# iyioon/NYPC-Yacht-Auction

Measured on AMD Instinct MI355X. Metric: MCTS node-expansions/sec/GPU @4096 envs x100 sims; episodes/sec 1-8 GPU, higher is better.
Workload: dtype f32

## Files before the change

nypc-yacht-auction_amd/csrc/yk_engine.hip:

```cpp
#include <math.h>

#include <algorithm>
#include <vector>

#include "yk_api.h"
#include "yk_common.h"
#include "yk_net.h"

#define YK_MAX_GROUPS 8

using namespace yk;

namespace {

constexpr int MAXD = 64;
constexpr int LUT_N = 1 << 16;
constexpr int GAMES_PER_BLOCK = 4;
constexpr int GROUP_ALIGN = 16;
constexpr int YK_EXPAND_WPE = 4;
constexpr int RO_CAP = 3072;
constexpr int RO_K = 512;
constexpr int RV_CAP = 1024;
constexpr uint32_t RV_OFF = 0xFFFFFFFFu;

enum : uint32_t { T_INT = 0, T_F64 = 1, T_F32 = 2 };

struct NodeRec {
    uint64_t key[8];
    uint64_t hash;
    uint64_t vinfo;
    uint32_t p_off;
    uint32_t nvalid;
    uint32_t Ns;
    uint32_t pad;
};
struct Edge {
    double Q;
    uint32_t N;
    uint32_t tag;
};
__device__ __forceinline__ uint32_t edge_kind(uint32_t tag) { return tag & 3u; }
constexpr uint32_t PATH_DET = 0x80000000u;

constexpr int GST = 16;
struct EngDev {
    int E, NCAP, HCAP, ECAP, M, VCAP;
    int e_lo, e_hi;
    int T, dual;
    int64_t AE;
    int sims, temp_threshold;
    float c32;
    int prior;
    int fparts;
    int rec_pred, max_exp, rec_stride;
    int arena;
    int arena_agent, arena_opp;
    uint64_t seed;
    NodeRec* nodes[2];
    uint32_t* hidx[2];
    Edge* edges[2];
    uint32_t* node_count;
    uint32_t* edge_count;
    float* arenaP;
    uint16_t* arenaS;
    uint32_t* arena_top;
    uint8_t* gen;
    uint8_t* cur_round;
    uint4* root_c;
    int ro_k;
    uint32_t* rv;
    uint16_t* ro_j;
    float* ro_p;
    yk_state_t* board;
    int32_t* cur;
    uint64_t* ctr;
    uint32_t* env_id;
    uint8_t* done;
    int32_t* nmoves;
    yk_state_t* root;
    int32_t* seat;
    uint8_t* idle;
    yk_state_t* leaf_state;
    uint64_t* leaf_hash;
    uint8_t* leaf_flag;
    uint64_t* path;
    uint8_t* path_len;
    uint32_t* end_node;
    double* res_v;
    uint32_t* res_t;
    const float* logits;
    const float* vpred;
    const float2* mlse;
    const float* lut_sq;
    const float* lut_sqe;
    yk_state_t* rec_state;
    int32_t* rec_info;
    uint64_t* rec_ctr;
    double* rec_val;
    uint32_t* rec_visits;
    int32_t* rec_voff;
    double* final_r;
    int32_t* final_cur;
    int32_t* final_tot;
    float* rec_pi;
    float* rec_v;
    yk_state_t* rec_leaf;
    uint64_t* gstats;
    uint32_t* err;
};

enum : uint32_t {
    ERR_NODES = 1u, ERR_EDGES = 2u, ERR_ARENA = 4u, ERR_DEPTH = 8u, ERR_STEP = 16u, ERR_ROUND = 32u,
    ERR_VISITS = 64u, ERR_MOVES = 128u, ERR_ZERO_COUNTS = 256u, ERR_ROOT = 512u, ERR_HASH = 1024u,
    ERR_FWD_SYNC = 2048u
};

struct PwPlan {
    int nleaf, nop, root;
    uint16_t start[64], len[64];
    uint8_t a[64], b[64];
};
constexpr int pw_build(PwPlan& p, int start, int n) {
    if (n <= 128) {
        p.start[p.nleaf] = (uint16_t)start;
        p.len[p.nleaf] = (uint16_t)n;
        return p.nleaf++;
    }
    int n2 = n / 2;
    n2 -= n2 % 8;
    const int l = pw_build(p, start, n2);
    const int r = pw_build(p, start + n2, n - n2);
    p.a[p.nop] = (uint8_t)l;
    p.b[p.nop] = (uint8_t)r;
    return 64 + p.nop++;
}
constexpr PwPlan make_plan() {
    PwPlan p{};
    p.root = pw_build(p, 0, ASIZE);
    return p;
}
static __constant__ PwPlan c_pw = make_plan();
static_assert(make_plan().nleaf <= 64 && make_plan().nop <= 64, "pairwise plan too large");
constexpr bool plan_is_butterfly() {
    const PwPlan p = make_plan();
    if (p.nleaf != 32 || p.nop != 31) return false;
    int first[128] = {}, cnt[128] = {};
    for (int i = 0; i < p.nleaf; i++) {
        if (p.start[i] % 8 != 0 || p.len[i] < 8 || p.len[i] > 128) return false;
        if (i > 0 && p.start[i] != p.start[i - 1] + p.len[i - 1]) return false;
        first[i] = i;
        cnt[i] = 1;
    }
    for (int o = 0; o < p.nop; o++) {
        const int a = p.a[o], b = p.b[o];
        if (cnt[a] != cnt[b] || first[a] + cnt[a] != first[b] || first[a] % (2 * cnt[a]) != 0) return false;
        first[64 + o] = first[a];
        cnt[64 + o] = 2 * cnt[a];
    }
    return p.root == 64 + p.nop - 1 && cnt[p.root] == 32;
}
static_assert(plan_is_butterfly(), "numpy's pairwise tree for 3226 is no longer a perfect 32-leaf tree");
constexpr int pw_gmax() {
    const PwPlan p = make_plan();
    int g = 0;
    for (int i = 0; i < p.nleaf; i++) g = p.len[i] / 8 > g ? p.len[i] / 8 : g;
    return g;
}
constexpr int pw_tmax() {
    const PwPlan p = make_plan();
    int t = 0;
    for (int i = 0; i < p.nleaf; i++) t = p.len[i] % 8 > t ? p.len[i] % 8 : t;
    return t;
}
constexpr int PW_GMAX = pw_gmax();
constexpr int PW_TMAX = pw_tmax() > 0 ? pw_tmax() : 1;

struct ValidQ {
    int mode;
    int n;
    uint32_t used;
    __device__ __forceinline__ bool operator()(int a) const {
        if (mode == 1) return a < NBID;
        if (mode != 0 || a < NBID) return false;
        const int base = a - NBID, cat = base / NCOMB, ci = base - cat * NCOMB;
        if ((used >> cat) & 1u) return false;
        if (n >= 10) return true;
        if (n == 5) return ci == 0;
        return c_tab.comb_max[ci] < n;
    }
};
__device__ __forceinline__ ValidQ valid_q(const YkS& s) {
    ValidQ q;
    const int round = s_round(s), phase = s_phase(s);
    const uint64_t wa = s_pw(s, 0, 0);
    q.n = __builtin_amdgcn_readfirstlane(wa_n(wa));
    q.used = __builtin_amdgcn_readfirstlane((uint32_t)wa_used(wa));
    q.mode = __builtin_amdgcn_readfirstlane((phase == 0 && round != 13) ? 1 : (phase == 1 && q.n >= 5) ? 0 : -1);
    return q;
}

__device__ __forceinline__ YkS ld_state(const yk_state_t* p) {
    const uint4* q = reinterpret_cast<const uint4*>(p);
    YkS s;
#pragma unroll
    for (int k = 0; k < 4; k++) {
        uint4 v = q[k];
        s.w[2 * k] = (uint64_t)v.x | ((uint64_t)v.y << 32);
        s.w[2 * k + 1] = (uint64_t)v.z | ((uint64_t)v.w << 32);
    }
    return s;
}
__device__ __forceinline__ void st_state(yk_state_t* p, const YkS& s) {
    uint4* q = reinterpret_cast<uint4*>(p);
#pragma unroll
    for (int k = 0; k < 4; k++)
        q[k] = make_uint4((uint32_t)s.w[2 * k], (uint32_t)(s.w[2 * k] >> 32), (uint32_t)s.w[2 * k + 1],
                          (uint32_t)(s.w[2 * k + 1] >> 32));
}
__device__ __forceinline__ bool key_eq(const NodeRec& r, const YkS& s) {
    bool eq = true;
#pragma unroll
// ... 176 lines not shown
    if (rr < cr) {
        if (lane == 0) atomicOr(d.err, ERR_ROUND);
        return;
    }
    const int g = d.gen[t], h = g ^ 1;
    uint32_t* hx = d.hidx[h] + (long)t * d.HCAP;
    for (int i = lane; i < d.HCAP; i += 64) hx[i] = 0;
    const NodeRec* src = d.nodes[g] + (long)t * d.NCAP;
    NodeRec* dst = d.nodes[h] + (long)t * d.NCAP;
    const Edge* esrc = d.edges[g] + (long)t * d.ECAP;
    Edge* edst = d.edges[h] + (long)t * d.ECAP;
    float* P = d.arenaP + (long)t * d.AE;
    uint16_t* S = d.arenaS + (long)t * d.AE;
    const uint32_t cnt = d.node_count[g * d.T + t];
    uint32_t nn = 0, ne = 0, top = 0;
    wave_sync();
    for (uint32_t b0 = 0; b0 < cnt; b0 += 64) {
    const uint32_t il = b0 + (uint32_t)lane;
    uint64_t live = __ballot(il < cnt && (int)(src[il < cnt ? il : 0].key[0] & 0xF) >= rr);
    while (live) {
        const uint32_t id = b0 + (uint32_t)__builtin_ctzll(live);
        live &= live - 1;
        NodeRec rec = src[id];
        const int V = (int)rec.nvalid, VP = pad4(V);
        const uint32_t so = rec.p_off;
        for (int j0 = 0; j0 < VP; j0 += 64) {
            const int j = j0 + lane;
            float p = 0.f;
            uint16_t sl = 0;
            if (j < VP) {
                p = P[so + j];
                sl = S[so + j];
            }
            const bool vis = j < V && sl != 0;
            const uint64_t bal = __ballot(vis);
            const uint32_t before = __popcll(bal & ((1ull << lane) - 1));
            uint16_t nsl = 0;
            if (vis) {
                Edge x = esrc[sl - 1];
                x.tag = edge_kind(x.tag);
                edst[ne + before] = x;
                nsl = (uint16_t)(ne + before + 1);
            }
            ne += (uint32_t)__popcll(bal);
            if (j < VP) {
                P[top + j] = p;
                S[top + j] = nsl;
            }
        }
        rec.p_off = top;
        top += (uint32_t)VP;
        if (lane == 0) {
            dst[nn] = rec;
            insert_index(d, h, t, rec.hash, nn);
        }
        nn++;
    }
    }
    if (lane == 0) {
        d.node_count[h * d.T + t] = nn;
        d.edge_count[h * d.T + t] = ne;
        d.arena_top[t] = top;
        d.gen[t] = (uint8_t)h;
        d.cur_round[t] = (uint8_t)rr;
    }
}


__device__ __forceinline__ int root_scan(const EngDev& d, int t, int lane, uint32_t nv, const float* P,
                                         const uint16_t* S, const Edge* edges, int V, int nk, int ws, float sq,
                                         float sqe, uint32_t& wtag, uint64_t& scanned, uint64_t& gathered) {
    const uint16_t* oj = d.ro_j + (long)t * RO_K;
    const float* op = d.ro_p + (long)t * RO_K;
    const uint32_t* rv = d.rv + (long)t * RV_CAP;
    int jj = ws + lane < nk ? (int)oj[ws + lane] : 0;
    float pp = ws + lane < nk ? op[ws + lane] : 0.f;
    float best = -INFINITY;
    int bj = 0x7FFFFFFF;
    uint32_t btag = 0;
    for (uint32_t i = (uint32_t)lane; i < nv; i += 64) {
        const uint32_t w = rv[i];
        const int j = (int)(w & 0xFFFu);
        const float p = P[j];
        const Edge ev = edges[(w >> 12) - 1];
        const float u = (float)ev.Q + ((d.c32 * p) * sq) / (float)(ev.N + 1);
        if (u > best || (u == best && j < bj)) {
            best = u;
            bj = j;
            btag = ev.tag;
        }
    }
    float ub = -INFINITY;
    int uj = 0x7FFFFFFF;
    bool found = false, done = false;
    int walked = 0;
    int first = nk;
    for (int k0 = ws; k0 < nk; k0 += 64) {
        const int k = k0 + lane;
        if (k0 != ws) {
            jj = k < nk ? (int)oj[k] : 0;
            pp = k < nk ? op[k] : 0.f;
        }
        walked = min(k0 + 64, nk) - ws;
        const bool in = k < nk;
        const bool unv = in && S[jj] == 0;
        const float u = (d.c32 * pp) * sqe;
        bool cand;
        if (!found) {
            const uint64_t bal = __ballot(unv);
            if (!bal) continue;
            const int f = __builtin_ctzll(bal);
            ub = lane_val(u, f);
            found = true;
            first = k0 + f;
            cand = unv && lane >= f && u == ub;
        } else {
            cand = unv && u == ub;
        }
        uj = min(uj, wave_min_i(cand ? jj : 0x7FFFFFFF));
        if (!(k0 + 64 < nk && lane_val(u, 63) == ub)) {
            done = k0 + 64 < nk || nk == V || lane_val(u, (nk - 1 - k0) & 63) != ub;
            break;
        }
    }
    if (lane == 0 && first != ws) d.root_c[2 * t + 1].w = (uint32_t)first;
    if (!done && nk < V) {
        scanned += (uint64_t)nv + (uint64_t)walked;
        gathered += (uint64_t)nv;
        return -1;
    }
    if (lane == 0 && found && (ub > best || (ub == best && uj < bj))) {
        best = ub;
        bj = uj;
        btag = 0;
    }
    const int mine = bj;
    wave_argmax_step(best, bj);
    const uint64_t own = __ballot(mine == bj);
    wtag = own ? __builtin_amdgcn_readlane(btag, (int)__builtin_ctzll(own)) : 0u;
    scanned += (uint64_t)nv + (uint64_t)walked;
    gathered += (uint64_t)nv;
    return bj;
}

__device__ __forceinline__ void select_game(const EngDev& d, int e, int lane, const uint32_t* env_ids, uint64_t* ctr_arr) {
    if (d.done[e] || d.idle[e]) {
        if (lane == 0) {
            d.leaf_flag[e] = 0;
            d.path_len[e] = 0;
            d.end_node[e] = 0;
        }
        return;
    }
    const int t = tree_of(d, e);
    const int g = d.gen[t];
    YkS s = ld_state(d.root + e);
    Stream rs{d.seed, env_ids[e], ctr_arr[e]};
    const NodeRec* nodes = d.nodes[g] + (long)t * d.NCAP;
    const Edge* edges = d.edges[g] + (long)t * d.ECAP;
    const float* Pbase = d.arenaP + (long)t * d.AE;
    const uint16_t* Sbase = d.arenaS + (long)t * d.AE;
    uint64_t* path = d.path + (long)e * MAXD;
    int depth = 0;
    uint64_t scanned = 0, gathered = 0;
    int ngl = 0;
    int leaf = 0;
    int known = -1;
    uint32_t end_id = 0;
    PyV res{0.0, T_INT};
    bool pre = false;
    int pre_bj = 0x7FFFFFFF;
    uint32_t pre_tag = 0;
    {
        const uint4 rc = d.root_c[2 * t], rc1 = d.root_c[2 * t + 1];
        if (rc.x != 0 && rc1.z != RV_OFF) {
            const uint32_t Ns = nodes[rc.x - 1].Ns;
            const float sq = (float)sqrt((double)Ns), sqe = (float)sqrt((double)Ns + 1e-8);
            pre_bj = __builtin_amdgcn_readfirstlane(root_scan(d, t, lane, rc1.z, Pbase + rc.y, Sbase + rc.y, edges,
                                                              (int)rc.z, (int)rc.w, (int)rc1.w, sq, sqe, pre_tag, scanned,
                                                              gathered));
            pre_tag = __builtin_amdgcn_readfirstlane(pre_tag);
            pre = pre_bj != -1;
        }
    }
    while (true) {
        if (known >= 0) {
            const uint64_t* kp = nodes[known].key;
#pragma unroll
            for (int i = 0; i < 8; i++) s.w[i] = kp[i];
        }
        const double es = game_ended(s, 1);
        if (es != 0.0) {
            res = PyV{-es, T_F64};
            break;
        }
        uint4 rc0 = make_uint4(0, 0, 0, 0), rc1 = rc0;
        if (depth == 0) {
            rc0 = d.root_c[2 * t];
            rc1 = d.root_c[2 * t + 1];
        }
        const bool cached = rc0.x != 0;
        const uint64_t hsh = (cached || known >= 0) ? 0ull : index_hash(s);
        const int nid = cached ? (int)rc0.x - 1 : known >= 0 ? known : lookup(d, g, t, s, hsh);
        if (nid < 0) {
            leaf = 1;
            if (lane == 0) {
                st_state(d.leaf_state + e, s);
                d.leaf_hash[e] = hsh;
            }
            break;
        }
        const NodeRec& nd = nodes[nid];
        const uint32_t p_off = cached ? rc0.y : nd.p_off;
        const int V = cached ? (int)rc0.z : (int)nd.nvalid;
        const uint64_t vinfo = cached ? ((uint64_t)rc1.x | ((uint64_t)rc1.y << 32)) : nd.vinfo;
        if (depth == 0 && !cached && lane == 0) {
            d.root_c[2 * t] = make_uint4((uint32_t)nid + 1, p_off, (uint32_t)V, 0);
            d.root_c[2 * t + 1] = make_uint4((uint32_t)vinfo, (uint32_t)(vinfo >> 32), RV_OFF, 0);
        }
        if (V == 0) {
            res = PyV{0.0, T_INT};
            end_id = (uint32_t)nid + 1;
            break;
        }
        const uint32_t Ns = nd.Ns;
        const float sq = (float)sqrt((double)Ns);
        const float sqe = (float)sqrt((double)Ns + 1e-8);
        const float* P = Pbase + p_off;
        const uint16_t* S = Sbase + p_off;
        int bj_out;
        uint32_t wtag;
        if (depth == 0 && pre) {
            bj_out = pre_bj;
            wtag = pre_tag;
        } else {
            float best = -INFINITY;
            int bj = 0x7FFFFFFF;
            uint32_t btag = 0;
            float4 p4 = make_float4(0.f, 0.f, 0.f, 0.f);
            ushort4 s4 = make_ushort4(0, 0, 0, 0);
            if (lane * 4 < V) {
                p4 = *reinterpret_cast<const float4*>(P + lane * 4);
                s4 = *reinterpret_cast<const ushort4*>(S + lane * 4);
            }
            for (int j0 = lane * 4; j0 < V; j0 += 256) {
                const float pv[4] = {p4.x, p4.y, p4.z, p4.w};
                const uint16_t sv[4] = {s4.x, s4.y, s4.z, s4.w};
                Edge ev[4];
#pragma unroll
                for (int t = 0; t < 4; t++)
                    if (j0 + t < V && sv[t]) {
                        ev[t] = edges[sv[t] - 1];
                        ngl++;
                    }
                if (j0 + 256 < V) {
                    p4 = *reinterpret_cast<const float4*>(P + j0 + 256);
                    s4 = *reinterpret_cast<const ushort4*>(S + j0 + 256);
                }
#pragma unroll
                for (int t = 0; t < 4; t++) {
                    const int j = j0 + t;
                    if (j < V) {
                        float u;
                        const float cp = d.c32 * pv[t];
                        if (sv[t]) {
                            u = (float)ev[t].Q + (cp * sq) / (float)(ev[t].N + 1);
                        } else {
                            u = cp * sqe;
                        }
                        if (u > best) {
                            best = u;
                            bj = j;
                            btag = sv[t] ? ev[t].tag : 0u;
                        }
                    }
                }
            }
            wave_argmax_step(best, bj);
            scanned += (uint64_t)V;
            bj_out = bj;
            wtag = __builtin_amdgcn_readlane(btag, __builtin_amdgcn_readfirstlane((bj & 255) >> 2));
        }
        const int bj = bj_out;
        int j = bj;
        if (j == 0x7FFFFFFF) j = 0;
        if (depth >= MAXD) {
            if (lane == 0) atomicOr(d.err, ERR_DEPTH);
            res = PyV{0.0, T_INT};
            break;
        }
        const uint32_t child = bj == 0x7FFFFFFF ? 0u : (wtag >> 2);
        if (child) {
            if (lane == 0) path[depth] = ((uint64_t)(p_off + (uint32_t)j) << 32) | (uint32_t)nid | PATH_DET;
            depth++;
            known = (int)child - 1;
            continue;
        }
        known = -1;
        const VInfo vi = unpack_vinfo(vinfo, (uint32_t)V);
        const int a = compact_to_action(vi, j);
        int np = 1;
        const uint64_t ctr0 = rs.ctr;
        const int st = step_state<true>(s, 1, a, rs, np);
        const uint32_t det = rs.ctr == ctr0 ? PATH_DET : 0u;
        if (lane == 0) path[depth] = ((uint64_t)(p_off + (uint32_t)j) << 32) | (uint32_t)nid | det;
        depth++;
        if (st != YK_ST_OK) {
            if (lane == 0) atomicOr(d.err, ERR_STEP);
            res = PyV{0.0, T_INT};
            break;
        }
        s = canonical(s, np);
    }
    gathered += (uint64_t)xlane_sum(ngl);
    if (lane == 0) {
        d.leaf_flag[e] = (uint8_t)(leaf ? (t < d.E ? 1 : 2) : 0);
        d.path_len[e] = (uint8_t)depth;
        d.end_node[e] = end_id;
        d.res_v[e] = res.v;
        d.res_t[e] = res.t;
        ctr_arr[e] = rs.ctr;
        d.gstats[(long)e * GST + 1] += scanned;
        d.gstats[(long)e * GST + 2] += (uint64_t)depth;
        d.gstats[(long)e * GST + 7] += 1;
        d.gstats[(long)e * GST + 8] += gathered;
    }
}

__global__ __launch_bounds__(256) __attribute__((amdgpu_waves_per_eu(4))) void k_select(EngDev d, const uint32_t* env_ids, uint64_t* ctr_arr) {
    const int lane = threadIdx.x & 63;
    const int e = d.e_lo + blockIdx.x * GAMES_PER_BLOCK + (threadIdx.x >> 6);
    if (e >= d.e_hi) return;
    select_game(d, e, lane, env_ids, ctr_arr);
}

__device__ __forceinline__ void expand_backup_game(const EngDev& d, int e, int lane);
__global__ __launch_bounds__(256) __attribute__((amdgpu_waves_per_eu(YK_EXPAND_WPE))) void k_expand_backup(
    EngDev d, int do_select, const uint32_t* env_ids, uint64_t* ctr_arr) {
    const int lane = threadIdx.x & 63;
    const int e = d.e_lo + blockIdx.x * GAMES_PER_BLOCK + (threadIdx.x >> 6);
    if (e >= d.e_hi) return;
    if (d.done[e]) return;
    expand_backup_game(d, e, lane);
    if (do_select) {
        wave_sync();
        select_game(d, e, lane, env_ids, ctr_arr);
    }
}

__device__ __forceinline__ void expand_backup_game(const EngDev& d, int e, int lane) {
    const int t = tree_of(d, e);
    const int g = d.gen[t];
    PyV res{d.res_v[e], d.res_t[e]};
    uint32_t end_id = 0;
    if (d.leaf_flag[e]) {
        const YkS s = ld_state(d.leaf_state + e);
        const uint64_t ihsh = d.leaf_hash[e];
        const uint64_t hsh = d.prior == 1 ? key_hash(s) : 0ull;
        const VInfo vi = valid_info(s, 1);
        const ValidQ valid = valid_q(s);
        const int V = vi.V;
        const int leaf = lane >> 1, h = lane & 1;
        const int st = c_pw.start[leaf], nl = c_pw.len[leaf], G = nl >> 3, R = nl & 7;
        float4 q[PW_GMAX];
        float qt[PW_TMAX];
        float v, mx = 0.f, lse = 0.f;
        const int pidx = (int)d.gstats[(long)e * GST + 0];
        const bool rec = d.rec_pred && (e % d.rec_stride) == 0 && pidx < d.max_exp;
        const long rslot = rec ? (long)(e / d.rec_stride) * d.max_exp + pidx : 0;
        bool masked = false;
        if (d.prior == 0) {
            const float* x = d.logits + (long)e * PI_LD + st;
            const float2 ml = d.mlse[e];
            mx = ml.x;
            lse = ml.y;
            if (d.fparts > 1) {
                float ms = ml.y;
                for (int p = 1; p < d.fparts; p++) {
                    const float2 q = d.mlse[(long)p * d.E + e];
                    const float mm = fmaxf(mx, q.x);
                    if (mm != -INFINITY) {
                        ms = ms * exp_acc(mx - mm) + q.y * exp_acc(q.x - mm);
                        mx = mm;
                    }
                }
                lse = logf(ms);
            }
            static_assert(NBID % 4 == 2 && NCOMB % 4 == 0, "category starts are 2 mod 4");
            const bool score10 = valid.mode == 0 && valid.n >= 10;
#pragma unroll
            for (int j = 0; j < PW_GMAX; j++) {
                const int a = st + 8 * j + 4 * h;
                bool v0, v1, v2, v3;
                if (score10) {
                    const int b0 = a - NBID, b2 = a + 2 - NBID;
                    const bool lo = j < G && b0 >= 0 && !((valid.used >> ((unsigned)b0 / NCOMB)) & 1u);
                    const bool hi = j < G && b2 >= 0 && !((valid.used >> ((unsigned)b2 / NCOMB)) & 1u);
                    v0 = v1 = lo;
                    v2 = v3 = hi;
                } else {
                    v0 = j < G && valid(a);
                    v1 = j < G && valid(a + 1);
                    v2 = j < G && valid(a + 2);
                    v3 = j < G && valid(a + 3);
                }
                float4 x4 = make_float4(0.f, 0.f, 0.f, 0.f);
                if (v0 || v1 || v2 || v3) x4 = *reinterpret_cast<const float4*>(x + 8 * j + 4 * h);
                q[j] = make_float4(v0 ? softmax_p(x4.x, mx, lse) : 0.f, v1 ? softmax_p(x4.y, mx, lse) : 0.f,
                                   v2 ? softmax_p(x4.z, mx, lse) : 0.f, v3 ? softmax_p(x4.w, mx, lse) : 0.f);
            }
#pragma unroll
            for (int r = 0; r < PW_TMAX; r++)
                qt[r] = (h == 0 && r < R && valid(st + 8 * G + r)) ? softmax_p(x[8 * G + r], mx, lse) : 0.f;
            v = d.vpred[e];
            masked = true;
        } else {
#pragma unroll
            for (int j = 0; j < PW_GMAX; j++) {
                const int a = st + 8 * j + 4 * h;
                q[j] = j < G ? make_float4(hash_prior_pi(hsh, a), hash_prior_pi(hsh, a + 1), hash_prior_pi(hsh, a + 2),
                                           hash_prior_pi(hsh, a + 3))
                             : make_float4(0.f, 0.f, 0.f, 0.f);
            }
#pragma unroll
            for (int r = 0; r < PW_TMAX; r++) qt[r] = (h == 0 && r < R) ? hash_prior_pi(hsh, st + 8 * G + r) : 0.f;
            v = hash_prior_v(hsh);
        }
#pragma unroll
        for (int j = 0; j < PW_GMAX; j++) {
            const int a = st + 8 * j + 4 * h;
            if (j < G && !masked) {
                if (!valid(a)) q[j].x = 0.f;
                if (!valid(a + 1)) q[j].y = 0.f;
                if (!valid(a + 2)) q[j].z = 0.f;
                if (!valid(a + 3)) q[j].w = 0.f;
            }
        }
#pragma unroll
        for (int r = 0; r < PW_TMAX; r++)
            if (h == 0 && r < R && !masked && !valid(st + 8 * G + r)) qt[r] = 0.f;
        if (rec) {
            float* rpi = d.rec_pi + rslot * ASIZE;
#pragma unroll
            for (int j = 0; j < PW_GMAX; j++)
                if (j < G) *reinterpret_cast<float4*>(rpi + st + 8 * j + 4 * h) = q[j];
#pragma unroll
            for (int r = 0; r < PW_TMAX; r++)
                if (h == 0 && r < R) rpi[st + 8 * G + r] = qt[r];
            if (lane == 0) {
                d.rec_v[rslot] = v;
                st_state(d.rec_leaf + rslot, s);
            }
        }
        float4 racc = q[0];
#pragma unroll
        for (int j = 1; j < PW_GMAX; j++)
            if (j < G) {
                racc.x += q[j].x;
                racc.y += q[j].y;
                racc.z += q[j].z;
                racc.w += q[j].w;
            }
        const float half = (racc.x + racc.y) + (racc.z + racc.w);
        const float other = xlane<1>(half);
        float lsum = h == 0 ? half + other : other + half;
#pragma unroll
        for (int r = 0; r < PW_TMAX; r++)
            if (r < R) lsum += qt[r];
        lsum = __builtin_bit_cast(float, dpp_mov<0xA0>(__builtin_bit_cast(uint32_t, lsum)));
        float y = xlane<2>(lsum);
        lsum = (lane & 2) ? y + lsum : lsum + y;
        y = xlane<4>(lsum);
        lsum = (lane & 4) ? y + lsum : lsum + y;
        y = xlane<8>(lsum);
        lsum = (lane & 8) ? y + lsum : lsum + y;
        y = xlane<16>(lsum);
        lsum = (lane & 16) ? y + lsum : lsum + y;
        y = xlane<32>(lsum);
        lsum = (lane & 32) ? y + lsum : lsum + y;
        const float sum = lsum;
        const int VP = pad4(V);
        const uint32_t off = d.arena_top[t];
        const uint32_t nid = d.node_count[g * d.T + t];
        bool ok = true;
        if ((int64_t)off + VP > d.AE) {
            if (lane == 0) atomicOr(d.err, ERR_ARENA);
            ok = false;
        }
        if (nid >= (uint32_t)d.NCAP) {
            if (lane == 0) atomicOr(d.err, ERR_NODES);
            ok = false;
        }
        if (ok) {
            float* P = d.arenaP + (long)t * d.AE + off;
            uint16_t* S = d.arenaS + (long)t * d.AE + off;
            const float inv_fallback = V > 0 ? 1.0f / (float)V : 0.0f;
            const float* __restrict__ xr = d.logits + (long)e * PI_LD;
            for (int j0 = lane; j0 < VP; j0 += 256) {
                float xa[4];
                int aa[4];
#pragma unroll
                for (int u = 0; u < 4; u++) {
                    const int j = j0 + 64 * u;
                    aa[u] = j < V ? compact_to_action(vi, j) : 0;
                    xa[u] = (d.prior == 0 && j < V) ? xr[aa[u]] : 0.f;
                }
#pragma unroll
                for (int u = 0; u < 4; u++) {
                    const int j = j0 + 64 * u;
                    if (j < VP) {
                        float p = 0.0f;
                        if (j < V) {
                            const float pa = d.prior == 0 ? softmax_p(xa[u], mx, lse) : hash_prior_pi(hsh, aa[u]);
                            p = sum > 0.0f ? pa / sum : inv_fallback;
                        }
                        P[j] = p;
                        S[j] = 0;
                    }
                }
            }
            if (lane == 0) {
                NodeRec r;
#pragma unroll
                for (int i = 0; i < 8; i++) r.key[i] = s.w[i];
                r.hash = ihsh;
                r.vinfo = pack_vinfo(vi);
                r.p_off = off;
                r.nvalid = (uint32_t)V;
                r.Ns = 0;
                r.pad = 0;
                d.nodes[g][(long)t * d.NCAP + nid] = r;
                if (!insert_index(d, g, t, ihsh, nid)) atomicOr(d.err, ERR_HASH);
            }
            end_id = nid + 1;
            if (lane == 0) {
                d.node_count[g * d.T + t] = nid + 1;
                d.arena_top[t] = off + (uint32_t)VP;
                uint64_t* gs = d.gstats + (long)e * GST;
                gs[0] += 1;
                gs[3] += (uint64_t)V;
                if (nid + 1 > gs[4]) gs[4] = nid + 1;
                if (off + VP > gs[6]) gs[6] = off + VP;
            }
        }
        res = PyV{-(double)v, T_F32};
    } else {
        end_id = d.end_node[e];
    }
    const int depth = d.path_len[e];
    if (depth > 0) {
        NodeRec* nodes = d.nodes[g] + (long)t * d.NCAP;
        Edge* edges = d.edges[g] + (long)t * d.ECAP;
        uint16_t* Sb = d.arenaS + (long)t * d.AE;
        const uint64_t* path = d.path + (long)e * MAXD;
        const uint32_t ne0 = d.edge_count[g * d.T + t];
        uint64_t pe = 0;
        uint16_t sl = 0;
        if (lane < depth) {
            pe = path[lane];
            sl = Sb[pe >> 32];
        }
        const uint32_t pnext = __shfl((uint32_t)pe, (lane + 1) & 63, 64);
        const uint32_t cnode = lane + 1 < depth ? (pnext & ~PATH_DET) + 1 : end_id;
        const uint32_t cbits = ((uint32_t)pe & PATH_DET) ? cnode << 2 : 0u;
        const bool is_new = lane < depth && sl == 0;
        const uint64_t bal = __ballot(is_new);
        const uint32_t eid = ne0 + (uint32_t)__popcll(bal & ((1ull << lane) - 1));
        const uint32_t ne1 = ne0 + (uint32_t)__popcll(bal);
        if (lane < depth) {
            PyV v = res;
            if ((depth - 1 - lane) & 1) v.v = -v.v;
            if (sl) {
                Edge& ed = edges[sl - 1];
                const PyV q = pv_update(PyV{ed.Q, edge_kind(ed.tag)}, ed.N, v);
                ed.Q = q.v;
                ed.tag = q.t | cbits;
                ed.N += 1;
            } else if (eid < (uint32_t)d.ECAP && eid < 65535u) {
                edges[eid] = Edge{v.v, 1u, v.t | cbits};
                Sb[pe >> 32] = (uint16_t)(eid + 1);
            } else {
                atomicOr(d.err, ERR_EDGES);
            }
            nodes[(uint32_t)pe & ~PATH_DET].Ns += 1;
        }
        if (lane == 0) {
            d.edge_count[g * d.T + t] = ne1;
            uint64_t* gs = d.gstats + (long)e * GST;
            if (ne1 > gs[5]) gs[5] = ne1;
            if (is_new && eid < (uint32_t)d.ECAP && eid < 65535u) {
                const uint32_t n = d.root_c[2 * t + 1].z;
                if (n != RV_OFF) {
                    const uint32_t j = (uint32_t)(pe >> 32) - d.root_c[2 * t].y;
                    if (n < (uint32_t)RV_CAP) {
                        d.rv[(long)t * RV_CAP + n] = j | ((eid + 1) << 12);
                        d.root_c[2 * t + 1].z = n + 1;
                    } else {
                        d.root_c[2 * t + 1].z = RV_OFF;
                    }
                }
            }
        }
    }
}

__global__ __launch_bounds__(256) void k_root_sort(EngDev d) {
    constexpr int PT = (RO_CAP + 255) / 256;
    __shared__ uint64_t sk[RO_K];
    __shared__ uint32_t hist[256];
    __shared__ int s_nid, s_need;
    __shared__ uint32_t s_nv, s_cnt;
    __shared__ uint64_t s_prefix;
    const int e = d.e_lo + (int)blockIdx.x;
    if (e >= d.e_hi || d.done[e] || d.idle[e] || !(d.c32 > 0.f)) return;
    const int tid = threadIdx.x, lane = tid & 63;
    const int t = tree_of(d, e);
    const int g = d.gen[t];
    const uint4 rc0 = d.root_c[2 * t];
    if (tid < 64) {
        int nid = rc0.x ? (int)rc0.x - 1 : -1;
        if (nid < 0) {
            const YkS r = ld_state(d.root + e);
            nid = lookup(d, g, t, r, index_hash(r));
        }
        if (tid == 0) {
            s_nid = nid;
            s_nv = 0;
            s_cnt = 0;
        }
    }
    __syncthreads();
    const int nid = s_nid;
    if (nid < 0) return;
    const NodeRec& nd = d.nodes[g][(long)t * d.NCAP + nid];
    const int V = (int)nd.nvalid;
    const uint32_t p_off = nd.p_off;
    if (V <= 256 || V > RO_CAP) return;
    const float* P = d.arenaP + (long)t * d.AE + p_off;
    const uint16_t* S = d.arenaS + (long)t * d.AE + p_off;
    uint32_t* rv = d.rv + (long)t * RV_CAP;
    uint64_t key[PT];
#pragma unroll
    for (int i = 0; i < PT; i++) {
        const int j = tid + 256 * i;
        key[i] = 0;
        if (j < V) {
            key[i] = ((uint64_t)__float_as_uint(P[j]) << 16) | (uint32_t)(0xFFFFu - (uint32_t)j);
            const uint16_t sl = S[j];
            if (sl) {
                const uint32_t pos = atomicAdd(&s_nv, 1u);
                if (pos < (uint32_t)RV_CAP) rv[pos] = (uint32_t)j | ((uint32_t)sl << 12);
            }
        }
    }
    const int K = V < d.ro_k ? V : d.ro_k;
    uint64_t thr = 1;
    if (V > K) {
        uint64_t prefix = 0, mask = 0;
        int need = K;
        for (int sh = 40; sh >= 0; sh -= 8) {
            hist[tid] = 0;
            __syncthreads();
#pragma unroll
            for (int i = 0; i < PT; i++)
                if (key[i] && (key[i] & mask) == prefix) atomicAdd(&hist[(uint32_t)(key[i] >> sh) & 255u], 1u);
            __syncthreads();
            if (tid < 64) {
                const uint32_t h0 = hist[4 * lane], h1 = hist[4 * lane + 1], h2 = hist[4 * lane + 2], h3 = hist[4 * lane + 3];
                const uint32_t own = h0 + h1 + h2 + h3;
                uint32_t suf = own;
#pragma unroll
                for (int o = 1; o < 64; o <<= 1) {
                    const uint32_t x = __shfl_down(suf, o, 64);
                    if (lane + o < 64) suf += x;
                }
                const uint32_t above = suf - own;
                if (above < (uint32_t)need && (uint32_t)need <= suf) {
                    const uint32_t hb[4] = {h0, h1, h2, h3};
                    uint32_t c = above;
                    int b = 3;
                    for (; b > 0; b--) {
                        if (c + hb[b] >= (uint32_t)need) break;
                        c += hb[b];
                    }
                    s_prefix = prefix | ((uint64_t)(4 * lane + b) << sh);
                    s_need = need - (int)c;
                }
            }
            __syncthreads();
            prefix = s_prefix;
            need = s_need;
            mask |= (uint64_t)255 << sh;
        }
        thr = prefix;
    }
#pragma unroll
    for (int i = 0; i < PT; i++)
        if (key[i] && key[i] >= thr) sk[atomicAdd(&s_cnt, 1u)] = key[i];
    int n2 = 64;
    while (n2 < K) n2 <<= 1;
    __syncthreads();
    for (int i = K + tid; i < n2; i += 256) sk[i] = 0;
    __syncthreads();
    for (int size = 2; size <= n2; size <<= 1) {
        for (int stride = size >> 1; stride > 0; stride >>= 1) {
            for (int i = tid; i < n2 / 2; i += 256) {
                const int lo = 2 * i - (i & (stride - 1)), hi = lo + stride;
                const bool desc = (lo & size) == 0;
                const uint64_t a = sk[lo], b = sk[hi];
                if ((a < b) == desc) {
                    sk[lo] = b;
                    sk[hi] = a;
                }
            }
            __syncthreads();
        }
    }
    uint16_t* oj = d.ro_j + (long)t * RO_K;
    float* op = d.ro_p + (long)t * RO_K;
    for (int i = tid; i < K; i += 256) {
        const uint64_t k = sk[i];
        oj[i] = (uint16_t)(0xFFFFu - (uint32_t)(k & 0xFFFFu));
        op[i] = __uint_as_float((uint32_t)(k >> 16));
    }
    if (tid == 0) {
        d.root_c[2 * t] = make_uint4((uint32_t)nid + 1, p_off, (uint32_t)V, (uint32_t)K);
        d.root_c[2 * t + 1] = make_uint4((uint32_t)nd.vinfo, (uint32_t)(nd.vinfo >> 32),
                                         s_nv <= (uint32_t)RV_CAP ? s_nv : RV_OFF, 0);
    }
}

__global__ __launch_bounds__(256) void k_move_end(EngDev d, int move) {
    __shared__ uint32_t vis_all[GAMES_PER_BLOCK][ASIZE];
    const int lane = threadIdx.x & 63, w = threadIdx.x >> 6;
    const int e = d.e_lo + blockIdx.x * GAMES_PER_BLOCK + w;
    if (e >= d.e_hi) return;
    if (d.done[e]) return;
    uint32_t* vis = vis_all[w];
    const int t = tree_of(d, e);
    const int g = d.gen[t];
    const YkS r = ld_state(d.root + e);
    const bool idle = d.idle[e] != 0;
// ... 324 lines not shown
            }
            if (timed) prof_mark(eng, g, KC_EXPAND, st[g]);
            const bool sort_root = k == 0 && sims > 1 && eng->root_scan;
            const bool fuse = k + 1 < sims && !sort_root;
            hipLaunchKernelGGL(k_expand_backup, game_grid(d), bb, 0, st[g], d, fuse && !eng->split_descent ? 1 : 0,
                               env_ids, ctr);
            YK_LAUNCHED();
            if (fuse && eng->split_descent) {
                hipLaunchKernelGGL(k_select, game_grid(d), bb, 0, st[g], d, env_ids, ctr);
                YK_LAUNCHED();
            }
            if (sort_root) {
                if (timed) prof_mark(eng, g, KC_SCAN, st[g]);
                hipLaunchKernelGGL(k_root_sort, dim3((unsigned)(d.e_hi - d.e_lo)), bb, 0, st[g], d);
                YK_LAUNCHED();
                hipLaunchKernelGGL(k_select, game_grid(d), bb, 0, st[g], d, env_ids, ctr);
                YK_LAUNCHED();
            }
            if (timed && eng->prof_stride > 1) prof_mark(eng, g, -1, st[g]);
        }
    }
    for (int g = 0; g < G; g++) prof_mark(eng, g, -1, st[g]);
    return YK_OK;
}
}

extern "C" {


int yk_engine_create(yk_engine_t** out, const yk_engine_config_t* cfg, yk_net_t* net) {
    if (!out || !cfg) return YK_ERR_ARG;
    if (cfg->n_envs <= 0 || cfg->sims < 1 || cfg->max_moves < 1 || cfg->max_moves > 4096) return YK_ERR_ARG;
    if (cfg->prior == 0 && !net) return YK_ERR_ARG;
    if (cfg->prior != 0 && cfg->prior != 1) return YK_ERR_ARG;
    yk_engine* eng = new yk_engine();
    eng->cfg = *cfg;
    eng->net = net;
    EngDev& d = eng->d;
    d.E = cfg->n_envs;
    d.sims = cfg->sims;
    d.c32 = (float)cfg->cpuct;
    d.temp_threshold = cfg->temp_threshold;
    d.prior = cfg->prior;
    d.M = cfg->max_moves;
    d.NCAP = 6 * cfg->sims + 64;
    int hcap = 1;
    while (hcap < 2 * d.NCAP) hcap <<= 1;
    d.HCAP = hcap;
    d.ECAP = std::min(4 * d.NCAP, 65535);
    if (cfg->arena_entries > 0) {
        d.AE = (cfg->arena_entries + 3) & ~3LL;
    } else {
        const int64_t worst = (int64_t)d.NCAP * 3024;
        size_t free_b = 0, total_b = 0;
        (void)hipMemGetInfo(&free_b, &total_b);
        const double need = (double)worst * 6.0 * cfg->n_envs * (cfg->dual_trees ? 2 : 1);
        d.AE = (need < 0.6 * (double)free_b) ? worst : (int64_t)cfg->sims * 9000 + 65536;
    }
    d.VCAP = (int)record_vcap(cfg->max_moves, cfg->sims);
    d.rec_pred = cfg->record_predictions ? 1 : 0;
    d.max_exp = cfg->record_predictions ? std::max(cfg->max_expansions, 1) : 0;
    d.rec_stride = std::max(cfg->record_stride, 1);
    d.e_lo = 0;
    d.e_hi = d.E;
    d.T = cfg->dual_trees ? 2 * d.E : d.E;
    d.dual = 0;
    eng->net2 = net;
    int G = cfg->groups > 0 ? cfg->groups : ((cfg->prior == 0 && cfg->n_envs >= 8192) ? 2 : 1);
    G = std::max(1, std::min({G, YK_MAX_GROUPS, (cfg->n_envs + GROUP_ALIGN - 1) / GROUP_ALIGN}));
    eng->ngroups = G;
constexpr int YK_FPARTS_MAX = 4;
    {
        int cus = 256, dev = 0;
        if (hipGetDevice(&dev) == hipSuccess) (void)hipDeviceGetAttribute(&cus, hipDeviceAttributeMultiprocessorCount, dev);
        const int tiles = G * (((cfg->n_envs + G - 1) / G + 15) / 16);
        d.fparts = 1;
        while (d.fparts * 2 <= YK_FPARTS_MAX && tiles * d.fparts * 2 <= cus) d.fparts *= 2;
        eng->fparts_single = d.fparts;
        if (cfg->dual_trees && G == 1 && cfg->prior == 0 && 2 * tiles <= cus) {
            eng->fparts_dual = 1;
            while (eng->fparts_dual * 2 <= YK_FPARTS_MAX && 2 * tiles * eng->fparts_dual * 2 <= cus) eng->fparts_dual *= 2;
        }
    }
    const size_t R = ((size_t)cfg->n_envs + d.rec_stride - 1) / d.rec_stride;
    const size_t E = (size_t)d.E, T = (size_t)d.T;
    int rc = YK_OK;
#define A(p, n) \
    if (rc == YK_OK) rc = dalloc(eng, &(p), (n))
    for (int g = 0; g < 2; g++) {
        A(d.nodes[g], T * d.NCAP);
        A(d.hidx[g], T * d.HCAP);
        A(d.edges[g], T * d.ECAP);
    }
    A(d.node_count, 2 * T);
    A(d.edge_count, 2 * T);
    A(d.arenaP, T * (size_t)d.AE);
    A(d.arenaS, T * (size_t)d.AE);
    A(d.arena_top, T);
    A(d.gen, T);
    A(d.cur_round, T);
    A(d.root_c, 2 * T);
    A(d.rv, T * RV_CAP);
    A(d.ro_j, T * RO_K);
    A(d.ro_p, T * RO_K);
    A(d.board, E);
    A(d.cur, E);
    A(d.ctr, E);
    A(d.env_id, E);
    A(d.done, E);
    A(d.nmoves, E);
    A(d.root, E);
    A(d.leaf_state, E);
    A(d.leaf_hash, E);
    A(d.leaf_flag, E);
    A(d.path, E * MAXD);
    A(d.path_len, E);
    A(d.end_node, E);
    A(d.res_v, E);
    A(d.res_t, E);
    A(eng->vpred, E);
    A(eng->mlse, E * (size_t)d.fparts);
    A(eng->lut_sq, (size_t)LUT_N);
    A(eng->lut_sqe, (size_t)LUT_N);
    A(d.rec_state, E * d.M);
    A(d.rec_info, E * d.M * 8);
    A(d.rec_ctr, E * d.M * 2);
    A(d.rec_val, E * d.M);
    A(d.rec_visits, E * (size_t)d.VCAP);
    A(d.rec_voff, E * (d.M + 1));
    A(d.final_r, E);
    A(d.final_cur, E);
    A(d.final_tot, 2 * E);
    A(d.seat, E);
    A(d.idle, E);
    A(d.gstats, E * GST);
    A(d.err, 1);
    A(eng->done_count, 1);
    A(eng->mcts_env, E);
    if (d.prior == 0) {
        A(eng->logits, E * (size_t)PI_LD);
    }
    if (d.rec_pred) {
        A(d.rec_pi, R * (size_t)d.max_exp * ASIZE);
        A(d.rec_v, R * (size_t)d.max_exp);
        A(d.rec_leaf, R * (size_t)d.max_exp);
    }
#undef A
    if (rc == YK_OK && hipHostMalloc((void**)&eng->host_done, sizeof(int32_t)) != hipSuccess) rc = YK_ERR_NOMEM;
    {
        const char* ev = getenv("YK_ROOT_SCAN");
        eng->root_scan = !(ev && ev[0] == '0');
        const char* ek = getenv("YK_ROOT_K");
        d.ro_k = ek ? std::max(1, std::min(RO_K, atoi(ek))) : RO_K;
        const char* es = getenv("YK_SPLIT_DESCENT");
        eng->split_descent = es && es[0] == '1';
    }
    if (rc == YK_OK && G > 1) {
        if (hipEventCreateWithFlags(&eng->ev_fork, hipEventDisableTiming) != hipSuccess) rc = YK_ERR_HIP;
        for (int g = 0; g < G && rc == YK_OK; g++)
            if (hipStreamCreateWithFlags(&eng->gs[g], hipStreamNonBlocking) != hipSuccess ||
                hipEventCreateWithFlags(&eng->ev_join[g], hipEventDisableTiming) != hipSuccess ||
                hipEventCreateWithFlags(&eng->ev_fwd[g], hipEventDisableTiming) != hipSuccess)
                rc = YK_ERR_HIP;
    }
    if (rc == YK_OK && eng->fparts_dual > 0) {
        if (hipStreamCreateWithFlags(&eng->dstream, hipStreamNonBlocking) != hipSuccess ||
            hipEventCreateWithFlags(&eng->ev_d0, hipEventDisableTiming) != hipSuccess ||
            hipEventCreateWithFlags(&eng->ev_d1, hipEventDisableTiming) != hipSuccess)
            rc = YK_ERR_HIP;
    }
    if (rc != YK_OK) {
        yk_engine_destroy(eng);
        return rc;
    }
    d.logits = eng->logits;
    d.vpred = eng->vpred;
    d.mlse = eng->mlse;
    d.lut_sq = eng->lut_sq;
    d.lut_sqe = eng->lut_sqe;
    hipLaunchKernelGGL(k_lut, dim3(LUT_N / 256), dim3(256), 0, 0, eng->lut_sq, eng->lut_sqe);
    YK_LAUNCHED();
    YK_HIP(hipMemset(d.err, 0, sizeof(uint32_t)));
    YK_HIP(hipMemset(d.done, 0, E));
    YK_HIP(hipMemset(d.idle, 0, E));
    YK_HIP(hipMemset(d.leaf_state, 0, sizeof(yk_state_t) * E));
    std::vector<uint32_t> ids(E);
    for (size_t i = 0; i < E; i++) ids[i] = (uint32_t)i;
    YK_HIP(hipMemcpy(eng->mcts_env, ids.data(), sizeof(uint32_t) * E, hipMemcpyHostToDevice));
    YK_HIP(hipDeviceSynchronize());
    *out = eng;
    return YK_OK;
}

int yk_engine_destroy(yk_engine_t* eng) {
    if (!eng) return YK_OK;
    for (auto& L : eng->pg)
        for (hipEvent_t e : L.ev) (void)hipEventDestroy(e);
    for (int g = 0; g < YK_MAX_GROUPS; g++) {
        if (eng->gs[g]) (void)hipStreamDestroy(eng->gs[g]);
        if (eng->ev_join[g]) (void)hipEventDestroy(eng->ev_join[g]);
        if (eng->ev_fwd[g]) (void)hipEventDestroy(eng->ev_fwd[g]);
    }
    if (eng->ev_fork) (void)hipEventDestroy(eng->ev_fork);
    if (eng->dstream) (void)hipStreamDestroy(eng->dstream);
    if (eng->ev_d0) (void)hipEventDestroy(eng->ev_d0);
    if (eng->ev_d1) (void)hipEventDestroy(eng->ev_d1);
    for (void* p : eng->allocs) (void)hipFree(p);
    if (eng->host_done) (void)hipHostFree(eng->host_done);
    delete eng;
    return YK_OK;
}

}

namespace {
int play_batch(yk_engine* eng, uint64_t seed, uint32_t env_base, hipStream_t s) {
    EngDev& d = eng->d;
    d.seed = seed;
    const int G = eng->ngroups;
    hipStream_t st[YK_MAX_GROUPS];
    EngDev dg[YK_MAX_GROUPS];
    for (int g = 0; g < G; g++) {
        st[g] = G == 1 ? s : eng->gs[g];
        dg[g] = G == 1 ? d : group_dev(eng, g);
    }
    const dim3 bb(256);
    YK_HIP(hipMemsetAsync(d.err, 0, sizeof(uint32_t), s));
    YK_HIP(hipMemsetAsync(d.hidx[0], 0, sizeof(uint32_t) * (size_t)d.T * d.HCAP, s));
    hipLaunchKernelGGL(k_reset, dim3((d.E + 255) / 256), dim3(256), 0, s, d, 1, env_base);
    YK_LAUNCHED();
    if (G > 1) {
        YK_HIP(hipEventRecord(eng->ev_fork, s));
        for (int g = 0; g < G; g++) YK_HIP(hipStreamWaitEvent(st[g], eng->ev_fork, 0));
    }
    eng->have_records = false;
    for (int move = 0; move < d.M; move++) {
        for (int g = 0; g < G; g++) {
            prof_mark(eng, g, KC_MOVE_BEGIN, st[g]);
            hipLaunchKernelGGL(k_move_begin, game_grid(dg[g]), bb, 0, st[g], dg[g], move, 0);
            YK_LAUNCHED();
        }
        if (!d.arena || d.arena_agent == YK_PLAYER_MCTS || d.arena_opp == YK_PLAYER_MCTS) {
            int rc = run_sims(eng, G, st, d.sims, d.env_id, d.ctr);
            if (rc) return rc;
        }
        for (int g = 0; g < G; g++) {
            prof_mark(eng, g, KC_MOVE_END, st[g]);
            hipLaunchKernelGGL(k_move_end, game_grid(dg[g]), bb, 0, st[g], dg[g], move);
            YK_LAUNCHED();
            prof_mark(eng, g, -1, st[g]);
            if (G > 1) {
                YK_HIP(hipEventRecord(eng->ev_join[g], st[g]));
                YK_HIP(hipStreamWaitEvent(s, eng->ev_join[g], 0));
            }
        }
        hipLaunchKernelGGL(k_count_done, dim3(1), dim3(1024), 0, s, d.done, d.E, eng->done_count);
        YK_LAUNCHED();
        YK_HIP(hipMemcpyAsync(eng->host_done, eng->done_count, sizeof(int32_t), hipMemcpyDeviceToHost, s));
        YK_HIP(hipStreamSynchronize(s));
        prof_collect(eng);
        if (*eng->host_done >= d.E) break;
    }
    hipLaunchKernelGGL(k_finalize, dim3((unsigned)(((long)d.E * d.M + 255) / 256)), dim3(256), 0, s, d);
    YK_LAUNCHED();
    eng->have_records = true;
    return check_errors(eng, s);
}
}

extern "C" {

int yk_selfplay(yk_engine_t* eng, uint64_t seed, uint32_t env_base, void* stream) {
    if (!eng) return YK_ERR_ARG;
    eng->d.arena = 0;
    eng->have_arena = false;
    return play_batch(eng, seed, env_base, as_stream(stream));
}

int yk_arena(yk_engine_t* eng, uint64_t seed, uint32_t env_base, const int32_t* agent_seat, int agent, int opponent,
             void* stream) {
    if (!eng || !agent_seat) return YK_ERR_ARG;
    if (agent < YK_PLAYER_MCTS || agent > YK_PLAYER_GREEDY || opponent < YK_PLAYER_MCTS || opponent > YK_PLAYER_GREEDY)
        return YK_ERR_ARG;
    EngDev& d = eng->d;
    for (int e = 0; e < d.E; e++)
        if (agent_seat[e] != 1 && agent_seat[e] != -1) return YK_ERR_ARG;
    hipStream_t s = as_stream(stream);
    YK_HIP(hipMemcpyAsync(d.seat, agent_seat, sizeof(int32_t) * (size_t)d.E, hipMemcpyHostToDevice, s));
    d.arena = 1;
    d.arena_agent = agent;
    d.arena_opp = opponent;
    d.dual = (d.T == 2 * d.E && agent == YK_PLAYER_MCTS && opponent == YK_PLAYER_MCTS) ? 1 : 0;
    if (d.dual && eng->dstream) d.fparts = eng->fparts_dual;
    eng->have_arena = false;
    const int rc = play_batch(eng, seed, env_base, s);
    d.arena = 0;
    d.dual = 0;
    d.fparts = eng->fparts_single;
    eng->have_arena = rc == YK_OK || rc == YK_ERR_STATE;
    return rc;
}

int yk_engine_set_opponent_net(yk_engine_t* eng, yk_net_t* net) {
    if (!eng || !net) return YK_ERR_ARG;
    if (eng->d.T != 2 * eng->d.E || eng->d.prior != 0) return YK_ERR_ARG;
    if (net->dev.H != eng->net->dev.H) return YK_ERR_ARG;
// ... 218 lines not shown
```

Before: 29.94 million.

## Cache first-visit argmax in node record to skip PUCT scan on unvisited nodes

During expansion, each new node computes the PUCT argmax for zero visits (prior-only scores) and stores it in the former padding field of the node record. Selection then reuses that index and skips the full child scan and wave reduction when a node's visit count is zero. A YK_NODE_SUMMARY env toggle controls this and defaults to on. Several wave-uniform values are made scalar with readfirstlane, and per-env stats updates become atomics, which adds atomic traffic to the stats writes.

Result: faster. 30.45 million (median of 6 runs) (+1.7%).

```diff
diff --git a/nypc-yacht-auction_amd/csrc/yk_engine.hip b/nypc-yacht-auction_amd/csrc/yk_engine.hip
--- a/nypc-yacht-auction_amd/csrc/yk_engine.hip
+++ b/nypc-yacht-auction_amd/csrc/yk_engine.hip
@@ -32,8 +32,9 @@
     uint32_t p_off;
     uint32_t nvalid;
     uint32_t Ns;
-    uint32_t pad;
+    uint32_t first_j;
 };
+static_assert(sizeof(NodeRec) == 96, "NodeRec: 96 bytes");
 struct Edge {
     double Q;
     uint32_t N;
@@ -67,6 +68,7 @@
     uint8_t* gen;
     uint8_t* cur_round;
     uint4* root_c;
+    int node_summary;
     int ro_k;
     uint32_t* rv;
     uint16_t* ro_j;
@@ -549,8 +551,8 @@
         }
         return;
     }
-    const int t = tree_of(d, e);
-    const int g = d.gen[t];
+    const int t = __builtin_amdgcn_readfirstlane(tree_of(d, e));
+    const int g = __builtin_amdgcn_readfirstlane((int)d.gen[t]);
     YkS s = ld_state(d.root + e);
     Stream rs{d.seed, env_ids[e], ctr_arr[e]};
     const NodeRec* nodes = d.nodes[g] + (long)t * d.NCAP;
@@ -634,30 +636,35 @@
             float best = -INFINITY;
             int bj = 0x7FFFFFFF;
             uint32_t btag = 0;
+            int Vs = V;
+            if (d.node_summary && Ns == 0) {
+                bj = (int)nd.first_j;
+                Vs = 0;
+            }
             float4 p4 = make_float4(0.f, 0.f, 0.f, 0.f);
             ushort4 s4 = make_ushort4(0, 0, 0, 0);
-            if (lane * 4 < V) {
+            if (lane * 4 < Vs) {
                 p4 = *reinterpret_cast<const float4*>(P + lane * 4);
                 s4 = *reinterpret_cast<const ushort4*>(S + lane * 4);
             }
-            for (int j0 = lane * 4; j0 < V; j0 += 256) {
+            for (int j0 = lane * 4; j0 < Vs; j0 += 256) {
                 const float pv[4] = {p4.x, p4.y, p4.z, p4.w};
                 const uint16_t sv[4] = {s4.x, s4.y, s4.z, s4.w};
                 Edge ev[4];
 #pragma unroll
                 for (int t = 0; t < 4; t++)
-                    if (j0 + t < V && sv[t]) {
+                    if (j0 + t < Vs && sv[t]) {
                         ev[t] = edges[sv[t] - 1];
                         ngl++;
                     }
-                if (j0 + 256 < V) {
+                if (j0 + 256 < Vs) {
                     p4 = *reinterpret_cast<const float4*>(P + j0 + 256);
                     s4 = *reinterpret_cast<const ushort4*>(S + j0 + 256);
                 }
 #pragma unroll
                 for (int t = 0; t < 4; t++) {
                     const int j = j0 + t;
-                    if (j < V) {
+                    if (j < Vs) {
                         float u;
                         const float cp = d.c32 * pv[t];
                         if (sv[t]) {
@@ -673,8 +680,8 @@
                     }
                 }
             }
-            wave_argmax_step(best, bj);
-            scanned += (uint64_t)V;
+            if (Vs) wave_argmax_step(best, bj);
+            scanned += (uint64_t)Vs;
             bj_out = bj;
             wtag = __builtin_amdgcn_readlane(btag, __builtin_amdgcn_readfirstlane((bj & 255) >> 2));
         }
@@ -717,16 +724,17 @@
         d.res_v[e] = res.v;
         d.res_t[e] = res.t;
         ctr_arr[e] = rs.ctr;
-        d.gstats[(long)e * GST + 1] += scanned;
-        d.gstats[(long)e * GST + 2] += (uint64_t)depth;
-        d.gstats[(long)e * GST + 7] += 1;
-        d.gstats[(long)e * GST + 8] += gathered;
+        unsigned long long* gs = reinterpret_cast<unsigned long long*>(d.gstats + (long)e * GST);
+        atomicAdd(gs + 1, (unsigned long long)scanned);
+        atomicAdd(gs + 2, (unsigned long long)depth);
+        atomicAdd(gs + 7, 1ull);
+        atomicAdd(gs + 8, (unsigned long long)gathered);
     }
 }
 
 __global__ __launch_bounds__(256) __attribute__((amdgpu_waves_per_eu(4))) void k_select(EngDev d, const uint32_t* env_ids, uint64_t* ctr_arr) {
     const int lane = threadIdx.x & 63;
-    const int e = d.e_lo + blockIdx.x * GAMES_PER_BLOCK + (threadIdx.x >> 6);
+    const int e = __builtin_amdgcn_readfirstlane(d.e_lo + blockIdx.x * GAMES_PER_BLOCK + (threadIdx.x >> 6));
     if (e >= d.e_hi) return;
     select_game(d, e, lane, env_ids, ctr_arr);
 }
@@ -735,7 +743,7 @@
 __global__ __launch_bounds__(256) __attribute__((amdgpu_waves_per_eu(YK_EXPAND_WPE))) void k_expand_backup(
     EngDev d, int do_select, const uint32_t* env_ids, uint64_t* ctr_arr) {
     const int lane = threadIdx.x & 63;
-    const int e = d.e_lo + blockIdx.x * GAMES_PER_BLOCK + (threadIdx.x >> 6);
+    const int e = __builtin_amdgcn_readfirstlane(d.e_lo + blockIdx.x * GAMES_PER_BLOCK + (threadIdx.x >> 6));
     if (e >= d.e_hi) return;
     if (d.done[e]) return;
     expand_backup_game(d, e, lane);
@@ -893,6 +901,9 @@
             uint16_t* S = d.arenaS + (long)t * d.AE + off;
             const float inv_fallback = V > 0 ? 1.0f / (float)V : 0.0f;
             const float* __restrict__ xr = d.logits + (long)e * PI_LD;
+            const float sqe0 = (float)sqrt((double)0u + 1e-8);
+            float fb = -INFINITY;
+            int fj = 0x7FFFFFFF;
             for (int j0 = lane; j0 < VP; j0 += 256) {
                 float xa[4];
                 int aa[4];
@@ -910,12 +921,18 @@
                         if (j < V) {
                             const float pa = d.prior == 0 ? softmax_p(xa[u], mx, lse) : hash_prior_pi(hsh, aa[u]);
                             p = sum > 0.0f ? pa / sum : inv_fallback;
+                            const float u0 = (d.c32 * p) * sqe0;
+                            if (u0 > fb) {
+                                fb = u0;
+                                fj = j;
+                            }
                         }
                         P[j] = p;
                         S[j] = 0;
                     }
                 }
             }
+            wave_argmax_step(fb, fj);
             if (lane == 0) {
                 NodeRec r;
 #pragma unroll
@@ -925,7 +942,7 @@
                 r.p_off = off;
                 r.nvalid = (uint32_t)V;
                 r.Ns = 0;
-                r.pad = 0;
+                r.first_j = (uint32_t)fj;
                 d.nodes[g][(long)t * d.NCAP + nid] = r;
                 if (!insert_index(d, g, t, ihsh, nid)) atomicOr(d.err, ERR_HASH);
             }
@@ -933,11 +950,11 @@
             if (lane == 0) {
                 d.node_count[g * d.T + t] = nid + 1;
                 d.arena_top[t] = off + (uint32_t)VP;
-                uint64_t* gs = d.gstats + (long)e * GST;
-                gs[0] += 1;
-                gs[3] += (uint64_t)V;
-                if (nid + 1 > gs[4]) gs[4] = nid + 1;
-                if (off + VP > gs[6]) gs[6] = off + VP;
+                unsigned long long* gs = reinterpret_cast<unsigned long long*>(d.gstats + (long)e * GST);
+                atomicAdd(gs + 0, 1ull);
+                atomicAdd(gs + 3, (unsigned long long)V);
+                atomicMax(gs + 4, (unsigned long long)(nid + 1));
+                atomicMax(gs + 6, (unsigned long long)(off + (uint32_t)VP));
             }
         }
         res = PyV{-(double)v, T_F32};
@@ -983,8 +1000,7 @@
         }
         if (lane == 0) {
             d.edge_count[g * d.T + t] = ne1;
-            uint64_t* gs = d.gstats + (long)e * GST;
-            if (ne1 > gs[5]) gs[5] = ne1;
+            atomicMax(reinterpret_cast<unsigned long long*>(d.gstats + (long)e * GST) + 5, (unsigned long long)ne1);
             if (is_new && eid < (uint32_t)d.ECAP && eid < 65535u) {
                 const uint32_t n = d.root_c[2 * t + 1].z;
                 if (n != RV_OFF) {
@@ -1615,6 +1631,8 @@
         eng->root_scan = !(ev && ev[0] == '0');
         const char* ek = getenv("YK_ROOT_K");
         d.ro_k = ek ? std::max(1, std::min(RO_K, atoi(ek))) : RO_K;
+        const char* en = getenv("YK_NODE_SUMMARY");
+        d.node_summary = (en && en[0] == '0') ? 0 : 1;
         const char* es = getenv("YK_SPLIT_DESCENT");
         eng->split_descent = es && es[0] == '1';
     }
```
